# Kakekakechan/AKBRaytracing

Hardware: AMD Instinct MI355X
Metric: ray-surface intersections/sec + PSF wall-time, 1e7-ray 4-mirror AKB, 1/2/4/8 GPU (higher is better)
Workload: dtype f64

## Files before the change

akbraytracing_amd/_lib.py:

```python
import atexit
import ctypes
import os

import torch

from . import build as _build

_LIB = None

c_i32 = ctypes.c_int32
c_i64 = ctypes.c_int64
c_int = ctypes.c_int
c_dbl = ctypes.c_double
c_vp = ctypes.c_void_p
MAX_MIRRORS = 7
ABI_VERSION = 19

FLAG_MISS = 0x1
FLAG_ZERO_NORMAL = 0x2
FLAG_ZERO_REFLECT = 0x4
FLAG_ZERO_DIR = 0x8
FLAG_CHAIN_DIR = 1 << 28
FLAG_FIG_OUTSIDE = 0x8

EXPORTS = [
    "akb_last_error", "akb_abi_version", "akb_sources_hash", "akb_device_count",
    "akb_stream_create_reserved", "akb_stream_destroy", "akb_reserved_cu_mask",
    "akb_isect_f64", "akb_normal_f64", "akb_reflect_f64", "akb_normalize_f64", "akb_plane_isect_f64",
    "akb_seglen_f64", "akb_rotate_f64", "akb_fill_nan_f64",
    "akb_isect_dd_f64", "akb_reflect_dd_f64", "akb_trace_chain_dd_f64", "akb_figure_opl_f64", "akb_figure_normal_f64",
    "akb_trace_chain_f64", "akb_chain_desc_size", "akb_tilt_opd_f64", "akb_tilt_params_f64",
    "akb_tilt_opd_dev_f64", "akb_chain_tilt_f64", "akb_chain_tilt_opd_f64", "akb_trace_chain_samples_f64", "akb_opd_f64", "akb_resample_f64", "akb_plane_sweep_rows_f64",
    "akb_plane_sweep_sink_f64",
    "akb_calc_ds_f64",
    "akb_pairwise_work_bytes", "akb_pairwise_sum_f64", "akb_pupil_sample_f64",
    "akb_leaf_sink_bytes", "akb_leaf_sink_layout", "akb_leaf_finish_work_bytes", "akb_leaf_finish_f64",
    "akb_leaf_parts_f64", "akb_parts_chain_f64",
    "akb_huygens_splits", "akb_huygens_work_bytes", "akb_huygens_f64", "akb_scale_field_f64",
    "akb_psf_work_bytes", "akb_psf_f64", "akb_psf_release_plans", "akb_release_all", "akb_selftest_arith_f64",
    "akb_first_valid_rows_f64", "akb_rotate_work_bytes", "akb_rotate_with_nan_f64", "akb_pupil_post_f64", "akb_pupil_post_work_bytes",
    "akb_moments_work_bytes", "akb_map_moments_f64", "akb_plane_subtract_f64", "akb_legendre_rows_f64",
    "akb_gd_cells_f64", "akb_gd_pockets", "akb_gd_check_pockets", "akb_gd_grad_sweeps_f64",
    "akb_gd_eval_f64", "akb_gd_cone_work_bytes", "akb_gd_patch_timing", "akb_gd_patch_times", "akb_gd_band_times", "akb_gd_patch_phases", "akb_gd_patch_order", "akb_gd_cone_eval_f64", "akb_gd_axes_f64",
    "akb_gd_cells_claims_f64", "akb_gd_claim_pockets_f64", "akb_gd_cone_solve_f64",
    "akb_gd_claims_f64", "akb_gd_cone_part_f64", "akb_gd_part_finish_f64", "akb_gd_ring_f64", "akb_gd_cells_window_f64",
    "akb_trace_chain_batch_f64", "akb_focus_eval_work_bytes", "akb_focus_eval_f64", "akb_sep_search_f64",
    "akb_finish_params_work_bytes", "akb_finish_tilt_params_f64",
    "akb_valid_mask_u8", "akb_external_contours", "akb_approx_poly_dp", "akb_affine_from_points",
    "akb_affine_invert", "akb_warp_affine_f64",
]


class LeafSink(ctypes.Structure):
    _fields_ = [
        ("leaf_sum", c_vp), ("leaf_cnt", c_vp), ("tail", c_vp),
        ("nq", c_i32), ("nan_mask", c_i32), ("n", c_i64),
    ]


class FigureMapDesc(ctypes.Structure):
    _fields_ = [
        ("table", c_vp),
        ("origin", c_dbl * 3), ("e_u", c_dbl * 3), ("e_w", c_dbl * 3),
        ("u0", c_dbl), ("du", c_dbl), ("w0", c_dbl), ("dw", c_dbl),
        ("nu", c_i32), ("nw", c_i32),
    ]

# ... 124 lines not shown
        "akb_gd_grad_sweeps_f64": ([c_vp, c_vp, c_int, c_int, c_vp, c_int, c_vp, c_vp, c_vp, c_vp, c_vp, c_vp, c_int,
                                    c_vp, c_vp, c_dbl, c_dbl, c_int, c_vp, c_vp, c_vp, c_vp, c_vp], c_int),
        "akb_gd_eval_f64": ([c_vp, c_vp, c_int, c_int, c_vp, c_int, c_vp, c_vp, c_vp, c_vp, c_int, c_vp, c_int,
                             c_vp, c_vp, c_int, c_vp, c_vp, c_vp], c_int),
        "akb_gd_cone_work_bytes": ([c_int, c_int, c_int, c_int, c_int], c_i64),
        "akb_gd_patch_timing": ([c_int], c_int),
        "akb_gd_patch_order": ([c_int, c_vp], c_int),
        "akb_gd_patch_times": ([c_vp, c_vp, c_int], c_int),
        "akb_gd_band_times": ([c_vp, c_int], c_int),
        "akb_gd_patch_phases": ([c_vp], c_int),
        "akb_gd_axes_f64": ([c_vp, c_vp, c_i64, c_int, c_int, c_vp, c_vp, c_vp, c_vp], c_int),
        "akb_gd_claims_f64": ([c_vp, c_vp, c_int, c_int, c_vp, c_int, c_vp, c_vp, c_vp, c_int, c_int, c_int, c_vp,
                               c_int, c_vp, c_int, c_vp, c_vp, c_vp], c_int),
        "akb_gd_cone_part_f64": ([c_vp, c_vp, c_int, c_int, c_vp, c_int, c_vp, c_vp, c_vp, c_vp, c_vp, c_i64, c_i64,
                                  c_int, c_vp, c_int, c_vp, c_int, c_vp, c_int, c_int, c_vp, c_vp, c_vp, c_vp, c_vp,
                                  c_vp, c_vp], c_int),
        "akb_gd_part_finish_f64": ([c_vp, c_vp, c_i64, c_int, c_vp], c_int),
        "akb_gd_ring_f64": ([c_vp, c_vp, c_int, c_int, c_vp, c_vp, c_vp, c_vp], c_int),
        "akb_gd_cells_window_f64": ([c_vp, c_vp, c_int, c_int, c_int, c_int, c_vp, c_dbl, c_vp, c_vp], c_int),
        "akb_gd_cone_eval_f64": ([c_vp, c_vp, c_int, c_int, c_vp, c_int, c_vp, c_vp, c_vp, c_vp, c_vp, c_vp, c_int,
                                  c_vp, c_int, c_vp, c_int, c_int, c_vp, c_vp, c_vp, c_vp, c_vp, c_vp], c_int),
        "akb_gd_cone_solve_f64": ([c_vp, c_vp, c_int, c_int, c_vp, c_int, c_vp, c_vp, c_vp, c_vp, c_vp, c_vp, c_int,
                                   c_vp, c_int, c_vp, c_int, c_int, c_vp, c_vp, c_vp, c_vp, c_vp, c_vp], c_int),
        "akb_gd_cells_claims_f64": ([c_vp, c_vp, c_int, c_int, c_vp, c_dbl, c_vp, c_vp, c_int, c_vp, c_int, c_vp,
                                     c_vp], c_int),
        "akb_gd_claim_pockets_f64": ([c_vp, c_vp, c_int, c_int, c_vp, c_int, c_vp, c_vp, c_int, c_vp, c_int, c_vp,
                                      c_vp], c_int),
    }
    for name, (args, res) in sig.items():
        try:
            f = getattr(L, name)
        except AttributeError:
            raise AKBError(f"the library lacks {name}: it was built from other sources, rebuild "
                           "(python -m akbraytracing_amd.build)") from None
        f.argtypes = args
        f.restype = res


def lib():
    global _LIB
    if _LIB is None:
        path = os.environ.get("AKB_LIB") or _build.SO
        if not os.path.exists(path):
            raise AKBError(
                f"{path} is missing: build the HIP extension first (python -m akbraytracing_amd.build "
                "or __graft_entry__.build()); there is no CPU fallback")
# ... 33 lines not shown
```

akbraytracing_amd/csrc/akb_griddata.hip:

```cpp
#include <hip/hip_runtime.h>
#include <math.h>
#include <stdint.h>
#include <stdio.h>

#include <algorithm>
#include <mutex>
#include <type_traits>

#include "akb_common.h"
#include "akb_pairwise.h"

namespace akb {
namespace {

struct Grid {
    const double* x;
    const double* y;
    int nv, nh;
    const uint8_t* diag;
    int npock;
    const int32_t* ptri;
    const int32_t* pnbr;
    const int32_t* edge_tri;
    const int32_t* xptr;
// ... 438 lines not shown
    }
    for (int off = 32; off > 0; off >>= 1) acc |= __shfl_down(acc, off);
    if (lane == 0) {
        const unsigned cur = __hip_atomic_load(flags, __ATOMIC_RELAXED, __HIP_MEMORY_SCOPE_AGENT);
        if ((cur | acc) != cur) atomicOr(flags, acc);
    }
}

__global__ void k_gd_ring(Grid g, double* rx, double* ry, unsigned* flags) {
    AKB_CHAIN_PRIORITY();
    const int64_t a = g.nh - 1, b = g.nv - 1, L = 2 * a + 2 * b;
    for (int64_t r = blockIdx.x * (int64_t)blockDim.x + threadIdx.x; r < L; r += (int64_t)gridDim.x * blockDim.x) {
        int64_t v;
        if (r < a) v = r;
        else if (r < a + b) v = (r - a) * g.nh + (g.nh - 1);
        else if (r < 2 * a + b) v = (int64_t)(g.nv - 1) * g.nh + (g.nh - 1 - (r - a - b));
        else v = (int64_t)(g.nv - 1 - (r - 2 * a - b)) * g.nh;
        rx[r] = g.x[v];
        ry[r] = g.y[v];
        if (!isfinite(rx[r]) || !isfinite(ry[r])) atomicOr(flags, 32u);
    }
}

__global__ void k_gd_check_pockets(Grid g, double tol, unsigned* flags) {
    AKB_CHAIN_PRIORITY();
    const int64_t nc2 = 2 * ncells(g);
    for (int64_t j = blockIdx.x * (int64_t)blockDim.x + threadIdx.x; j < g.npock; j += (int64_t)gridDim.x * blockDim.x) {
        const Tri T = tri_verts(g, nc2 + j);
        for (int k = 0; k < 3; ++k) {
            const int64_t n = tri_nbr(g, nc2 + j, k);
            if (n < 0) continue;
            const Tri N = tri_verts(g, n);
            int64_t o = -1;
            for (int q = 0; q < 3; ++q)
                if (N.v[q] != T.v[(k + 1) % 3] && N.v[q] != T.v[(k + 2) % 3]) o = N.v[q];
            if (o < 0) {
                atomicOr(flags, 4u);
                continue;
            }
            const double x0 = g.x[T.v[0]], y0 = g.y[T.v[0]];
            const double bx = g.x[T.v[1]] - x0, by = g.y[T.v[1]] - y0, cx = g.x[T.v[2]] - x0, cy = g.y[T.v[2]] - y0;
            const double ox = g.x[o] - x0, oy = g.y[o] - y0;
            const double s = fmax(fmax(fabs(bx), fabs(by)), fmax(fmax(fabs(cx), fabs(cy)), fmax(fabs(ox), fabs(oy))));
            if (incircle(0.0, 0.0, bx, by, cx, cy, ox, oy) > tol * s * s * s * s) atomicOr(flags, 2u);
        }
    }
}


__device__ __forceinline__ int64_t ring_pos(const Grid& g, int iv, int ih) {
    const int64_t a = g.nh - 1, b = g.nv - 1;
    if (iv == 0) return ih;
    if (ih == g.nh - 1) return a + iv;
    if (iv == g.nv - 1) return a + b + (g.nh - 1 - ih);
    if (ih == 0) return 2 * a + b + (g.nv - 1 - iv);
    return -1;
}

__device__ __forceinline__ int64_t ring_vertex(const Grid& g, int64_t r) {
    const int64_t ra = g.nh - 1, rb = g.nv - 1;
    if (r < ra) return r;
    if (r < ra + rb) return (r - ra) * g.nh + (g.nh - 1);
    if (r < 2 * ra + rb) return (int64_t)(g.nv - 1) * g.nh + (g.nh - 1 - (r - ra - rb));
    return (int64_t)(g.nv - 1 - (r - 2 * ra - rb)) * g.nh;
}

struct EdgeG {
    double mxx, mxy, myy, wx, wy;
};
// ... 688 lines not shown
        int32_t* sr = slots + r * kChordSlots;
        for (int k = 0; k < kChordSlots; ++k)
            sr[k] = cnt > kChordSlots ? kSlotBig
                    : k >= cnt        ? -1
                    : cnt > 8         ? -g.xidx[k0 + k] - 3
                                      : g.xidx[k0 + k];
    }
}

constexpr int kBandThreads = 256, kBandRingWaves = kBandThreads / 64, kBandRingPer = 8 * kBandRingWaves;
constexpr int kBandTileThreads = kBandThreads, kBandVR = kBandTR * kBandTC / kBandTileThreads;
__device__ __forceinline__ void band_clock(unsigned long long* clk, int k, unsigned long long t0) {
    __syncthreads();
    if (threadIdx.x == 0) {
        const unsigned long long d = wall_clock64() - t0;
        atomicAdd(&clk[2 * k], d);
        atomicAdd(&clk[2 * k + 1], 1ull);
        atomicMax(&clk[4 + k], d);
    }
}
inline unsigned band_ring_wgs(int64_t L) { return (unsigned)((L + kBandRingPer - 1) / kBandRingPer); }
inline unsigned band_grid(const BandTiles& bt, int64_t L) { return band_ring_wgs(L) + (unsigned)bt.total; }

__global__ void __launch_bounds__(kBandThreads) __attribute__((amdgpu_waves_per_eu(4))) k_gd_cone_band(Grid g, BandTiles bt, ConeBand a) {
    AKB_CHAIN_PRIORITY();
    if (!*a.needed) return;
    const unsigned long long t0 = a.clk ? wall_clock64() : 0;
    constexpr int HR = kBandTR + 2, HC = kBandTC + 2, HN = HR * HC, CC = kBandTC + 1;
    __shared__ double sx[HN], sy[HN], sf[HN], sgx[HN], sgy[HN];
    __shared__ double spx[kBandTR * kBandTC], spy[kBandTR * kBandTC];
    __shared__ uint8_t sdg[(kBandTR + 1) * CC];
    const int64_t L = 2 * (int64_t)(g.nh - 1) + 2 * (int64_t)(g.nv - 1);
    const int nr = (int)((L + kBandRingPer - 1) / kBandRingPer);
    const int w = threadIdx.x >> 6, lane = threadIdx.x & 63;
    if ((int)blockIdx.x < nr) {
        const int sub = lane & 7;
        const int64_t q0 = (int64_t)blockIdx.x * kBandRingPer + 8 * w;
        const int64_t r = q0 + (lane >> 3);
        int32_t js[4] = {-1, -1, -1, -1};
        bool big;
        if (a.slots) {
            if (r < L) {
#pragma unroll
                for (int k = 0; k < 4; ++k) js[k] = a.slots[r * kChordSlots + sub + 8 * k];
            }
            big = js[0] == kSlotBig;
        } else {
            big = r < L && g.xptr[r + 1] - g.xptr[r] > 8;
        }
        if (r < L && !big) cone_ring_vertex<8>(g, a, r, sub, js);
        unsigned long long m = __ballot(big && sub == 0);
        while (m) {
            const int q = __builtin_ctzll(m);
            m &= m - 1;
            cone_ring_vertex<64>(g, a, q0 + (q >> 3), lane);
        }
        if (a.clk) band_clock(a.clk + 4, 0, t0);
        return;
    }
    int r0 = 0, c0 = 0, r1 = 0, c1 = 0;
    band_tile(bt, g.nv, g.nh, (int)blockIdx.x - nr, r0, c0, r1, c1);
    {
        constexpr int NQ = (HN + kBandThreads - 1) / kBandThreads, NC = ((kBandTR + 1) * CC + kBandThreads - 1) / kBandThreads;
        constexpr int NP = kBandTR * kBandTC / kBandThreads;
        double lx[NQ], ly[NQ], lf[NQ], lgx[NQ], lgy[NQ], lpx[NP], lpy[NP];
        uint8_t ld[NC];
#pragma unroll
        for (int u = 0; u < NQ; ++u) {
            const int k = threadIdx.x + u * kBandThreads;
            const int iv = r0 - 1 + k / HC, ih = c0 - 1 + (k - (k / HC) * HC);
            lx[u] = ly[u] = lf[u] = lgx[u] = lgy[u] = 0.0;
            if (k < HN && iv >= 0 && iv < g.nv && ih >= 0 && ih < g.nh) {
                const int64_t q = (int64_t)iv * g.nh + ih;
                lx[u] = g.x[q];
                ly[u] = g.y[q];
                lf[u] = a.f[q];
                lgx[u] = a.gin ? a.gin[2 * q] : 0.0;
                lgy[u] = a.gin ? a.gin[2 * q + 1] : 0.0;
            }
        }
#pragma unroll
        for (int u = 0; u < NC; ++u) {
            const int k = threadIdx.x + u * kBandThreads;
            const int cv = r0 - 1 + k / CC, ch = c0 - 1 + (k - (k / CC) * CC);
// ... 49 lines not shown
        const int lc = tr * CC + tc;
        const int dc[4] = {lc, lc + 1, lc + CC, lc + CC + 1};
        uint8_t dg[4];
#pragma unroll
        for (int k = 0; k < 4; ++k) dg[k] = inb[4 + k] ? sdg[dc[k]] : 0;
        double xs[8], ys[8], fs[8], gxs[8], gys[8];
#pragma unroll
        for (int k = 0; k < 8; ++k) {
            const int j = inb[k] ? jn[k] : li;
            xs[k] = sx[j];
            ys[k] = sy[j];
            fs[k] = sf[j];
            gxs[k] = sgx[j];
            gys[k] = sgy[j];
        }
        const bool on[8] = {L_, R, D, U, inb[4] && dg[0] == 0, inb[5] && dg[1] == 1, inb[6] && dg[2] == 1,
                            inb[7] && dg[3] == 0};
        GradAcc<1> A;
        band_edges(A, sx[li], sy[li], sf[li], xs, ys, fs, gxs, gys, on);
        const int pk = tr * kBandTC + tc;
        band_solve(a, (int64_t)iv * g.nh + ih, A, spx[pk], spy[pk]);
    }
    if (a.clk) band_clock(a.clk + 4, 1, t0);
}

struct ConePatch {
    const double* f;
    const int64_t* cells;
    const int* count;
    int K;
    ConeStep st[kConeMaxK + 1];
    double* gout;
    unsigned long long* chg;
    unsigned long long* est;
    unsigned long long* clk;
};

__constant__ uint16_t c_patch_order[kConeMaxK + 1][1024];

inline int b128_lane_group(int lane) {
    const int x = lane & 31;
    const bool first = x < 4 || (x >= 12 && x < 16) || (x >= 20 && x < 28);
    return (lane >> 5) * 2 + (first ? 0 : 1);
}

inline void patch_order_table(int K, int S, uint16_t* out) {
// ... 446 lines not shown
    __shared__ PwTree tree[2];
    __threadfence_block();
    __syncthreads();
    const int w = threadIdx.x >> 6;
    if (w < 2) {
        const long long cnt = (long long)mx * my;
        const double* a = lds ? (w == 0 ? sgx : sgy) : (w == 0 ? gx : gy);
        const int m = w == 0 ? mx : my;
        double sum;
        sum = pw_sum_wave_get(tree[w], MeshgridAxis{a, mx, w == 0}, cnt);
        const double mean = sum / (double)cnt;
        if ((threadIdx.x & 63) == 0) ext[4 + w] = m > 1 ? fabs((a[1] - mean) - (a[0] - mean)) : 0.0;
    }
}

__device__ __forceinline__ bool cone_interior(const Grid& g, int o, int K, int64_t& c, int64_t& p00) {
    if (o >= 2 * ncells(g)) return false;
    c = o >> 1;
    const int iv = (int)(c / (g.nh - 1)), ih = (int)(c - (int64_t)iv * (g.nh - 1));
    p00 = (int64_t)iv * g.nh + ih;
    return iv - K - 1 >= 1 && iv + K + 2 <= g.nv - 2 && ih - K - 1 >= 1 && ih + K + 2 <= g.nh - 2;
}

__global__ void __launch_bounds__(kBlock) k_gd_cone_assign(Grid g, const int* __restrict__ owner, int64_t m, int K,
                                                            int64_t own0, int64_t own1, int band_on, int64_t* cells,
                                                            int* count, int* band, uint8_t* assigned) {
    AKB_CHAIN_PRIORITY();
    for (int64_t t = blockIdx.x * (int64_t)blockDim.x + threadIdx.x; t < m; t += (int64_t)gridDim.x * blockDim.x) {
        const int o = owner[t];
        uint8_t mine = 0;
        if (o != INT32_MAX) {
            int64_t c = -1, p00 = -1;
            const bool interior = cone_interior(g, o, K, c, p00);
            if (interior) {
                if (p00 >= own0 && p00 < own1) {
                    cells[atomicAdd(count, 1)] = c;
                    mine = 1;
                }
            } else if (band_on) {
                atomicOr(band, 1);
                mine = 1;
            }
        }
        assigned[t] = mine;
    }
}

__global__ void __launch_bounds__(kBlock) k_gd_claim(Grid g, Targets t, int* owner) {
    AKB_CHAIN_PRIORITY();
    const int64_t ntri = 2 * ncells(g);
    for (int64_t id = blockIdx.x * (int64_t)blockDim.x + threadIdx.x; id < ntri; id += (int64_t)gridDim.x * blockDim.x) {
        const Tri T = tri_verts(g, id);
        int c0, c1, r0, r1;
        tri_box(g, t, T, c0, c1, r0, r1);
        for (int r = r0; r < r1; ++r)
            for (int c = c0; c < c1; ++c) claim_one(g, t, T, (int)id, r, c, owner);
    }
}

__device__ __forceinline__ void claim_cell(const Grid& g, const Targets& t, int64_t c, bool uniform, double inv_dx,
                                           double inv_dy, int* owner) {
    const int iv = (int)(c / (g.nh - 1)), ih = (int)(c - (int64_t)iv * (g.nh - 1));
    const int64_t p00 = (int64_t)iv * g.nh + ih;
    const double xa = g.x[p00], xb = g.x[p00 + 1], xc = g.x[p00 + g.nh], xd = g.x[p00 + g.nh + 1];
    const double ya = g.y[p00], yb = g.y[p00 + 1], yc = g.y[p00 + g.nh], yd = g.y[p00 + g.nh + 1];
    const double xlo = fmin(fmin(xa, xb), fmin(xc, xd)), xhi = fmax(fmax(xa, xb), fmax(xc, xd));
    const double ylo = fmin(fmin(ya, yb), fmin(yc, yd)), yhi = fmax(fmax(ya, yb), fmax(yc, yd));
    const double padx = (xhi - xlo) * 1e-9, pady = (yhi - ylo) * 1e-9;
// ... 159 lines not shown
    Targets tl = t;
    if (t.mx <= kClaimAxisLds && t.my <= kClaimAxisLds) {
        for (int i = threadIdx.x; i < t.mx; i += blockDim.x) sax[i] = t.gx[i];
        for (int i = threadIdx.x; i < t.my; i += blockDim.x) sax[kClaimAxisLds + i] = t.gy[i];
        __syncthreads();
        tl.gx = sax;
        tl.gy = sax + kClaimAxisLds;
    }
    const int lane = threadIdx.x & 63, wv = threadIdx.x >> 6, nw = blockDim.x >> 6;
    int64_t nblk;
    int bh, r_lo, r_hi;
    claim_block_dims(g, nblk, bh, r_lo, r_hi);
    for (int64_t blk = (int64_t)blockIdx.x * nw + wv; blk < nblk; blk += (int64_t)gridDim.x * nw) {
        if (!hit[blk]) continue;
        const int bv = (int)(blk / bh), bc = (int)(blk - (int64_t)bv * bh);
        const int iv0 = r_lo + bv * 8, ih0 = bc * 8;
        const int nr = min(8, r_hi - iv0), nc = min(8, g.nh - 1 - ih0);
        const int rr = lane >> 3, cc = lane & 7;
        if (rr < nr && cc < nc) claim_cell(g, tl, (int64_t)(iv0 + rr) * (g.nh - 1) + (ih0 + cc), uniform, inv_dx, inv_dy,
                                           owner);
    }
}

__global__ void __launch_bounds__(kBlock) k_gd_claim_pockets(Grid g, Targets t, int* owner) {
    AKB_CHAIN_PRIORITY();
    const int64_t nc2 = 2 * ncells(g);
    const int lane = threadIdx.x & 63, nw = blockDim.x >> 6;
    __shared__ double sax[2 * kClaimAxisLds];
    if (t.mx <= kClaimAxisLds && t.my <= kClaimAxisLds) {
        for (int i = threadIdx.x; i < t.mx; i += blockDim.x) sax[i] = t.gx[i];
        for (int i = threadIdx.x; i < t.my; i += blockDim.x) sax[kClaimAxisLds + i] = t.gy[i];
        __syncthreads();
        t.gx = sax;
        t.gy = sax + kClaimAxisLds;
    }
    for (int64_t j = (int64_t)blockIdx.x * nw + (threadIdx.x >> 6); j < g.npock; j += (int64_t)gridDim.x * nw) {
        const Tri T = tri_verts(g, nc2 + j);
        int c0, c1, r0, r1;
        tri_box(g, t, T, c0, c1, r0, r1);
        const int w = c1 - c0;
        const int64_t m = (int64_t)w * (r1 - r0);
        for (int64_t k = lane; k < m; k += 64) {
            const int r = r0 + (int)(k / w), c = c0 + (int)(k - (int64_t)(k / w) * w);
            claim_one(g, t, T, (int)(nc2 + j), r, c, owner);
        }
    }
}

struct CTIn {
    double px[3], py[3], f[3], gx[3], gy[3];
    double cx[3], cy[3];
    bool nb[3];
};

__device__ __forceinline__ void bary_v(const double (&x)[3], const double (&y)[3], double px, double py,
                                       double (&b)[3]) {
    const double x2 = x[2], y2 = y[2];
    const double a00 = x[0] - x2, a01 = x[1] - x2;
    const double a10 = y[0] - y2, a11 = y[1] - y2;
    const double det = a00 * a11 - a01 * a10;
    const double t00 = a11 / det, t01 = -a01 / det, t10 = -a10 / det, t11 = a00 / det;
    const double dx = px - x2, dy = py - y2;
    b[0] = t00 * dx + t01 * dy;
    b[1] = t10 * dx + t11 * dy;
    b[2] = 1.0 - b[0] - b[1];
}

__device__ double ct_eval(const CTIn& in, const double (&b)[3]) {
    const double p0x = in.px[0], p0y = in.py[0];
// ... 414 lines not shown
    AKB_REQUIRE(ring_x && ring_y && gx && gy && L > 0 && mx > 0 && my > 0, "bad arguments");
    k_gd_axes<<<1, kAxesThreads, 0, (hipStream_t)stream>>>(ring_x, ring_y, L, mx, my, gx, gy, d_extent);
    return launch_status("k_gd_axes");
}


static int64_t claim_scratch_bytes(int nv, int nh) {
    return ((int64_t)((nv - 1 + 7) / 8) * ((nh - 1 + 7) / 8) + 63) / 64 * 64;
}
static int64_t claim_scratch_offset(int nv, int nh, int mx, int my, int nvals) {
    const int64_t n = (int64_t)nv * nh, L = 2 * (int64_t)(nh - 1) + 2 * (int64_t)(nv - 1);
    const int nv2 = nvals >= 2 ? 2 : 1;
    const int64_t m = (int64_t)mx * my;
    return (3 * (int64_t)nv2 * n * 2 * 8 + L * 16 * 8 + m * 8 + m + 64 + 63) / 64 * 64;
}

int64_t akb_gd_cone_work_bytes(int nv, int nh, int mx, int my, int nvals) {
    if (nv < 2 || nh < 2 || mx < 1 || my < 1 || nvals < 1) return -1;
    return claim_scratch_offset(nv, nh, mx, my, nvals) + claim_scratch_bytes(nv, nh);
}

namespace {

int cone_claims(const Grid& g, const Targets& t, int with_pockets, int* owner, hipStream_t s, uint8_t* scratch = nullptr) {
    const int64_t m = (int64_t)t.mx * t.my;
    k_fill_i32<<<grid_for(m, 4), kBlock, 0, s>>>(owner, m, INT32_MAX);
    int st = launch_status("k_fill_i32");
    if (st) return st;
    const int64_t wc = (int64_t)((g.row1 < 0 ? g.nv - 1 : g.row1) - g.row0) * (g.nh - 1);
    if (wc > 0) {
        if (scratch) {
            const int64_t nblk = (int64_t)(((g.row1 < 0 ? g.nv - 1 : g.row1) - g.row0 + 7) / 8) * ((g.nh - 1 + 7) / 8);
            k_gd_claim_scan<<<grid_for(nblk, 1, kStreamGridCap), kBlock, 0, s>>>(g, t, scratch);
            if ((st = launch_status("k_gd_claim_scan"))) return st;
            k_gd_claim_hit<<<grid_for(nblk * 16, 1, kStreamGridCap), kBlock, 0, s>>>(g, t, scratch, owner);
        } else {
            k_gd_claim_blocks<<<grid_for(wc / 16 + 1, 1, kStreamGridCap), kBlock, 0, s>>>(g, t, owner);
        }
        if ((st = launch_status("k_gd_claim"))) return st;
    }
    if (with_pockets && g.npock > 0) {
        const int64_t pw = ((int64_t)g.npock + kBlock / 64 - 1) / (kBlock / 64);
        k_gd_claim_pockets<<<(unsigned)(pw < 16384 ? pw : 16384), kBlock, 0, s>>>(g, t, owner);
        if ((st = launch_status("k_gd_claim_pockets"))) return st;
    }
    return 0;
}

int cone_part(const Grid& g, const Targets& t, int64_t own0, int64_t own1, int band_on, const double* f, int nvals,
              int K, const double* omegas, void* work, const int* owner, double* out, double* cnt,
              unsigned long long* d_change, hipStream_t s) {
    const int64_t n = (int64_t)g.nv * g.nh, m = (int64_t)t.mx * t.my;
    const int64_t L = 2 * (int64_t)(g.nh - 1) + 2 * (int64_t)(g.nv - 1);
    double* gb[3];
    for (int k = 0; k < 3; ++k) gb[k] = (double*)work + (int64_t)k * n * 2;
    const int nv2 = nvals >= 2 ? 2 : 1;
    int64_t* cells = (int64_t*)((double*)work + 3 * (int64_t)nv2 * n * 2 + L * 16);
    uint8_t* assigned = (uint8_t*)(cells + m);
    int* count = (int*)(((uintptr_t)(assigned + m) + 7) & ~(uintptr_t)7);
    int* band = count + 1;
    if (hipMemsetAsync(count, 0, 2 * sizeof(int), s) != hipSuccess) return launch_status("hipMemsetAsync");
    k_gd_cone_assign<<<grid_for(m, 1), kBlock, 0, s>>>(g, owner, m, K, own0, own1, band_on, cells, count, band,
                                                      assigned);
    int st = launch_status("k_gd_cone_assign");
    if (st) return st;
    ConeStep steps[kConeMaxK + 1];
    steps[0] = ConeStep{0, 1.0};
    for (int j = 1; j <= K; ++j)
        steps[j] = j == 1 ? ConeStep{0, 1.0} : j == 2 ? ConeStep{1, omegas[1]} : ConeStep{2, omegas[j - 1]};
    const int S = patch_split(K);
    const unsigned pp = gd_cu_count();
    AKB_REQUIRE(S >= 0 && m <= 1024 * (int64_t)pp, "cone patches: K or the target count out of range");
    if (patch_order_upload(s)) {
        set_error("cone patches: the vertex order table did not reach constant memory");
        return AKB_E_HIP;
    }
    for (int v = 0; v < nvals; ++v) {
        const double* fv = f + v * n;
        if (band_on) {
            PatchTimer& bt0 = patch_timer();
            const int bslot = (int)(bt0.band_launches % kPatchEvents);
            if (bt0.on) (void)hipEventRecord(bt0.bev[bslot][0], s);
            int32_t* slots = (int32_t*)((double*)work + 3 * (int64_t)nv2 * n * 2);
            if (v == 0) {
                k_gd_chord_slots<<<grid_for(L), kBlock, 0, s>>>(g, slots, L);
                if ((st = launch_status("k_gd_chord_slots"))) return st;
            }
            for (int j = 1; j <= K; ++j) {
                const double* gin = j == 1 ? nullptr : gb[(j - 1) % 3];
                const double* gprev = j >= 3 ? gb[(j + 1) % 3] : nullptr;
                const BandTiles bt = band_tiles(g.nv, g.nh, 2 * K + 3 - j);
                const ConeBand a{fv, gin, gprev, gb[j % 3], steps[j], band, patch_timer().band_clk ? patch_timer().clk : nullptr,
                                 slots};
                k_gd_cone_band<<<band_grid(bt, L), kBandThreads, 0, s>>>(g, bt, a);
                if ((st = launch_status("k_gd_cone_band"))) return st;
            }
            if (d_change) {
                const BandTiles bt = band_tiles(g.nv, g.nh, K + 2);
                const ConeBand a{fv, gb[K % 3], nullptr, gb[(K + 1) % 3], ConeStep{0, 1.0}, band,
                                 patch_timer().band_clk ? patch_timer().clk : nullptr, slots};
                k_gd_cone_band<<<band_grid(bt, L), kBandThreads, 0, s>>>(g, bt, a);
                if ((st = launch_status("k_gd_cone_band"))) return st;
            }
            if (bt0.on) {
                (void)hipEventRecord(bt0.bev[bslot][1], s);
                ++bt0.band_launches;
            }
        }
        const BandEst be{band_on && d_change ? gb[(K + 1) % 3] : nullptr, K, d_change, d_change ? d_change + 1 : nullptr};
        ConePatch a{fv, cells, count, K, {}, gb[K % 3], d_change, d_change ? d_change + 1 : nullptr,
                    patch_timer().on ? patch_timer().clk : nullptr};
        for (int j = 0; j <= K; ++j) a.st[j] = steps[j];
        PatchTimer& pt = patch_timer();
        const int slot = (int)(pt.launches % kPatchEvents);
        if (pt.on) {
            (void)hipEventRecord(pt.ev[slot][0], s);
            pt.cnt[slot] = count;
// ... 64 lines not shown
    const int64_t pw = ((int64_t)npock + kBlock / 64 - 1) / (kBlock / 64);
    k_gd_claim_pockets<<<(unsigned)(pw < 16384 ? pw : 16384), kBlock, 0, (hipStream_t)stream>>>(g, Targets{gx, gy, mx, my},
                                                                                               owner);
    return launch_status("k_gd_claim_pockets");
}

int akb_gd_cone_solve_f64(const double* x, const double* y, int nv, int nh, const uint8_t* diag, int npock,
                          const int32_t* ptri, const int32_t* pnbr, const int32_t* edge_tri, const int32_t* xptr,
                          const int32_t* xidx, const double* gx, int mx, const double* gy, int my, const double* f,
                          int nvals, int K, const double* omegas, void* work, const int* owner, double* out,
                          unsigned long long* d_change, void* stream) {
    clear_error();
    AKB_REQUIRE(x && y && diag && gx && gy && f && omegas && work && owner && out && mx > 0 && my > 0 && nvals >= 1,
                "bad arguments");
    AKB_REQUIRE(K >= 1 && K <= kConeMaxK, "K sweeps in 1 .. 14");
    AKB_REQUIRE(nv >= 2 && nh >= 2, "grid of at least 2 x 2 points");
    AKB_REQUIRE(xptr && xidx && (npock == 0 || (ptri && pnbr && edge_tri)), "the band needs the pockets");
    for (int j = 2; j <= K; ++j) AKB_REQUIRE(omegas[j - 1] > 0 && omegas[j - 1] < 2, "Chebyshev weight outside (0, 2)");
    Grid g{x, y, nv, nh, diag, npock, ptri, pnbr, edge_tri, xptr, xidx};
    return cone_part(g, Targets{gx, gy, mx, my}, 0, (int64_t)nv * nh, 1, f, nvals, K, omegas, work, owner, out, nullptr,
                     d_change, (hipStream_t)stream);
}

int akb_gd_claims_f64(const double* x, const double* y, int nv, int nh, const uint8_t* diag, int npock,
                      const int32_t* ptri, const int32_t* pnbr, const int32_t* edge_tri, int row0, int row1,
                      int with_pockets, const double* gx, int mx, const double* gy, int my, int* owner, void* work,
                      void* stream) {
    clear_error();
    AKB_REQUIRE(x && y && diag && gx && gy && owner && mx > 0 && my > 0, "bad arguments");
    AKB_REQUIRE(nv >= 2 && nh >= 2 && row0 >= 0 && row1 <= nv - 1 && (row1 < 0 || row0 <= row1), "bad window");
    AKB_REQUIRE(!with_pockets || npock == 0 || (ptri && pnbr && edge_tri), "pockets needed");
    Grid g{x, y, nv, nh, diag, npock, ptri, pnbr, edge_tri, nullptr, nullptr};
    g.row0 = row0;
    g.row1 = row1;
    return cone_claims(g, Targets{gx, gy, mx, my}, with_pockets, owner, (hipStream_t)stream,
                       work ? (uint8_t*)work + claim_scratch_offset(nv, nh, mx, my, 1) : nullptr);
}

int akb_gd_cone_part_f64(const double* x, const double* y, int nv, int nh, const uint8_t* diag, int npock,
                         const int32_t* ptri, const int32_t* pnbr, const int32_t* edge_tri, const int32_t* xptr,
                         const int32_t* xidx, int64_t own0, int64_t own1, int band_on, const double* gx, int mx,
                         const double* gy, int my, const double* f, int nvals, int K, const double* omegas, void* work,
                         const int* owner, double* out, double* cnt, unsigned long long* d_change, void* stream) {
    clear_error();
    AKB_REQUIRE(x && y && diag && gx && gy && f && omegas && work && owner && out && cnt && mx > 0 && my > 0,
                "bad arguments");
// ... 124 lines not shown
```

akbraytracing_amd/faithful.py:

```python
import concurrent.futures
import time

import numpy as np
import torch

from . import _lib
from . import device as D
from .griddata import CONE_GUARD, CONE_SWEEPS, ConeNotConverged, CubicGrid, build_pockets, chebyshev_weights
from .griddata import pocket_offsets, raise_for_cell_flags, raise_for_pocket_status
from .psf import image_axes, psf_stack
from .pupilmap import POST_PARAMS, pupil_post, pupil_post_check

EUV = 13.5e-9


def pack_pockets(buf, o, Lr):
    npk = int(buf[o["npk"]])
    nx = int(buf[o["xptr"] + Lr])
    nbr = buf[o["nbr"]:o["nbr"] + 3 * npk].copy()
    rest = np.concatenate([buf[o["edge"]:o["edge"] + Lr], buf[o["xptr"]:o["xptr"] + Lr + 1],
                           buf[o["xidx"]:o["xidx"] + nx]])
    p = dict(tri=0, nbr=3 * npk, edge=6 * npk, xptr=6 * npk + Lr, xidx=6 * npk + 2 * Lr + 1)
    assert o["tri"] == 0
    buf[p["nbr"]:p["nbr"] + 3 * npk] = nbr
# ... 202 lines not shown
            t.npock = D.wait_result(t.job)
        except BaseException:
            t.y = t.z = t.f = None
            t.finished = True
            raise
        s = t.slot
        st = stream_of(stream)
        sh = D.stream_handle(st)
        o, Lr = s["po"], self.L
        with torch.cuda.stream(st):
            if self._done is not None:
                st.wait_event(self._done)
            if events is not None:
                events[0].record(st)
            s["pk"][:o["len"]].copy_(s["pk_host"][:o["len"]], non_blocking=True)
            t.h2d = torch.cuda.Event()
            t.h2d.record(st)
            pk = s["pk"]
            k = max(t.npock, 1)
            ptri, pnbr = pk[o["tri"]:o["tri"] + 3 * k], pk[o["nbr"]:o["nbr"] + 3 * k]
            edge, xptr, xidx = pk[o["edge"]:o["edge"] + Lr], pk[o["xptr"]:o["xptr"] + Lr + 1], pk[o["xidx"]:o["len"] + 1]
            tri = (D.ptr(t.y), D.ptr(t.z), self.nv, self.nh, D.ptr(s["diag"]), t.npock, D.ptr(ptri), D.ptr(pnbr),
                   D.ptr(edge))
            self.words[:3].zero_()
            _lib.check(L.akb_gd_check_pockets(*tri, self.tol, D.ptr(self.status), sh))
            m = self.size
            axes = s["axes"]
            gx, gy = axes[:m], axes[m:2 * m]
            _lib.check(L.akb_gd_claim_pockets_f64(D.ptr(t.y), D.ptr(t.z), self.nv, self.nh, D.ptr(s["diag"]), t.npock,
                                                  D.ptr(ptri), D.ptr(gx), m, D.ptr(gy), m, D.ptr(s["owner"]), sh))
            _lib.check(L.akb_gd_cone_solve_f64(*tri, D.ptr(xptr), D.ptr(xidx), D.ptr(gx), m, D.ptr(gy), m,
                                               D.ptr(t.f), 1, self.sweeps, self._omegas, D.ptr(self.work),
                                               D.ptr(s["owner"]), D.ptr(self.map), D.ptr(self.change), sh))
            t.result = self._post_psf(st, axes, psf_events, post_events)
            if events is not None:
                events[1].record(st)
            t.erow = self.errors.record((self.words,), st)
            t.done = self._end(st)
        t.y = t.z = t.f = None
        t.finished = True
        self.finished += 1
        return t.result

    def run(self, y, z, f, stream=None):
        t = self.begin(y, z, f, stream)
        r = self.finish(t, stream)
        try:
            t.check()
        except ConeNotConverged:
            r = self._converged(y, z, f, t.slot["axes"], stream)
        return r

    def _converged(self, y, z, f, ax, stream=None):
        st = stream_of(stream)
        m = self.size
        with torch.cuda.stream(st):
# ... 16 lines not shown
```

include/akb_raytrace.h:

```cpp
#ifndef AKB_RAYTRACE_H
#define AKB_RAYTRACE_H

#include <stdint.h>

#ifdef __cplusplus
extern "C" {
#endif

#define AKB_ABI_VERSION 19

#define AKB_OK 0
#define AKB_E_INVALID (-1)
#define AKB_E_HIP (-2)
#define AKB_E_FFT (-3)
#define AKB_E_NOMEM (-4)
#define AKB_E_ARG AKB_E_INVALID

#define AKB_FLAG_MISS 0x1
#define AKB_FLAG_ZERO_NORMAL 0x2
#define AKB_FLAG_ZERO_REFLECT 0x4
#define AKB_FLAG_ZERO_DIR 0x8
#define AKB_FLAG_CHAIN_DIR (1 << 28)
#define AKB_FLAG_FIG_OUTSIDE 0x8

// ... 240 lines not shown
int akb_gd_patch_timing(int enable);
int akb_gd_patch_times(float* ms, int* cells, int max);
int akb_gd_band_times(float* ms, int max);
int akb_gd_patch_phases(unsigned long long* out);
int akb_gd_patch_order(int K, uint16_t* out);
int akb_gd_axes_f64(const double* ring_x, const double* ring_y, int64_t L, int mx, int my, double* gx, double* gy,
                    double* d_extent, void* stream);
int akb_gd_cone_eval_f64(const double* x, const double* y, int nv, int nh, const uint8_t* diag, int npock,
                         const int32_t* ptri, const int32_t* pnbr, const int32_t* edge_tri, const int32_t* xptr,
                         const int32_t* xidx, const double* gx, int mx, const double* gy, int my, const double* f,
                         int nvals, int K, const double* omegas, void* work, int* owner, double* out,
                         unsigned long long* d_change, void* stream);
int akb_gd_cells_claims_f64(const double* x, const double* y, int nv, int nh, uint8_t* diag, double tol,
                            unsigned* d_flags, const double* gx, int mx, const double* gy, int my, int* owner,
                            void* stream);
int akb_gd_claim_pockets_f64(const double* x, const double* y, int nv, int nh, const uint8_t* diag, int npock,
                             const int32_t* ptri, const double* gx, int mx, const double* gy, int my, int* owner,
                             void* stream);
int akb_gd_cone_solve_f64(const double* x, const double* y, int nv, int nh, const uint8_t* diag, int npock,
                          const int32_t* ptri, const int32_t* pnbr, const int32_t* edge_tri, const int32_t* xptr,
                          const int32_t* xidx, const double* gx, int mx, const double* gy, int my, const double* f,
                          int nvals, int K, const double* omegas, void* work, const int* owner, double* out,
                          unsigned long long* d_change, void* stream);

int akb_gd_cells_window_f64(const double* x, const double* y, int nv, int nh, int row0, int row1, uint8_t* diag,
                            double tol, unsigned* d_flags, void* stream);
int akb_gd_ring_f64(const double* x, const double* y, int nv, int nh, double* ring_x, double* ring_y, unsigned* d_flags,
                    void* stream);
int akb_gd_claims_f64(const double* x, const double* y, int nv, int nh, const uint8_t* diag, int npock,
                      const int32_t* ptri, const int32_t* pnbr, const int32_t* edge_tri, int row0, int row1,
                      int with_pockets, const double* gx, int mx, const double* gy, int my, int* owner, void* work,
                      void* stream);
int akb_gd_cone_part_f64(const double* x, const double* y, int nv, int nh, const uint8_t* diag, int npock,
                         const int32_t* ptri, const int32_t* pnbr, const int32_t* edge_tri, const int32_t* xptr,
                         const int32_t* xidx, int64_t own0, int64_t own1, int band_on, const double* gx, int mx,
                         const double* gy, int my, const double* f, int nvals, int K, const double* omegas, void* work,
                         const int* owner, double* out, double* cnt, unsigned long long* d_change, void* stream);
int akb_gd_part_finish_f64(double* out, const double* cnt, int64_t m, int nvals, void* stream);

#define AKB_SELFTEST_COLS 13
int akb_selftest_arith_f64(const double* a, const double* b, int64_t n, double* out, void* stream);

void akb_psf_release_plans(void);

void akb_release_all(void);

// ... 6 lines not shown
```

Before: 58.79 billion.

## Fold pocket check, pocket claims and cone assign into leading band-sweep launches

Adds a cone_finish entry point that merges the pocket-consistency check, pocket claiming, chord-slot fill, status/count zeroing and cone assignment into extra leading workgroups of the first two k_gd_cone_band launches. Python now calls this single entry instead of three separate library calls. The aim is to remove several small kernel launches and memsets, and the gaps between them, on the griddata path. In exchange the band kernels carry a templated lead path, and the code relies on the work in each launch being independent. The claims in launch 1 must finish before the assign in launch 2 reads the owner array, which kernel order on the stream provides.

```diff
diff --git a/akbraytracing_amd/_lib.py b/akbraytracing_amd/_lib.py
--- a/akbraytracing_amd/_lib.py
+++ b/akbraytracing_amd/_lib.py
@@ -42,7 +42,7 @@
     "akb_moments_work_bytes", "akb_map_moments_f64", "akb_plane_subtract_f64", "akb_legendre_rows_f64",
     "akb_gd_cells_f64", "akb_gd_pockets", "akb_gd_check_pockets", "akb_gd_grad_sweeps_f64",
     "akb_gd_eval_f64", "akb_gd_cone_work_bytes", "akb_gd_patch_timing", "akb_gd_patch_times", "akb_gd_band_times", "akb_gd_patch_phases", "akb_gd_patch_order", "akb_gd_cone_eval_f64", "akb_gd_axes_f64",
-    "akb_gd_cells_claims_f64", "akb_gd_claim_pockets_f64", "akb_gd_cone_solve_f64",
+    "akb_gd_cells_claims_f64", "akb_gd_claim_pockets_f64", "akb_gd_cone_solve_f64", "akb_gd_cone_finish_f64",
     "akb_gd_claims_f64", "akb_gd_cone_part_f64", "akb_gd_part_finish_f64", "akb_gd_ring_f64", "akb_gd_cells_window_f64",
     "akb_trace_chain_batch_f64", "akb_focus_eval_work_bytes", "akb_focus_eval_f64", "akb_sep_search_f64",
     "akb_finish_params_work_bytes", "akb_finish_tilt_params_f64",
@@ -213,6 +213,9 @@
                                   c_vp, c_int, c_vp, c_int, c_int, c_vp, c_vp, c_vp, c_vp, c_vp, c_vp], c_int),
         "akb_gd_cone_solve_f64": ([c_vp, c_vp, c_int, c_int, c_vp, c_int, c_vp, c_vp, c_vp, c_vp, c_vp, c_vp, c_int,
                                    c_vp, c_int, c_vp, c_int, c_int, c_vp, c_vp, c_vp, c_vp, c_vp, c_vp], c_int),
+        "akb_gd_cone_finish_f64": ([c_vp, c_vp, c_int, c_int, c_vp, c_int, c_vp, c_vp, c_vp, c_vp, c_vp, c_dbl, c_vp,
+                                    c_vp, c_int, c_vp, c_int, c_vp, c_int, c_int, c_vp, c_vp, c_vp, c_vp, c_vp, c_vp],
+                                   c_int),
         "akb_gd_cells_claims_f64": ([c_vp, c_vp, c_int, c_int, c_vp, c_dbl, c_vp, c_vp, c_int, c_vp, c_int, c_vp,
                                      c_vp], c_int),
         "akb_gd_claim_pockets_f64": ([c_vp, c_vp, c_int, c_int, c_vp, c_int, c_vp, c_vp, c_int, c_vp, c_int, c_vp,
diff --git a/akbraytracing_amd/csrc/akb_griddata.hip b/akbraytracing_amd/csrc/akb_griddata.hip
--- a/akbraytracing_amd/csrc/akb_griddata.hip
+++ b/akbraytracing_amd/csrc/akb_griddata.hip
@@ -484,10 +484,9 @@
     }
 }
 
-__global__ void k_gd_check_pockets(Grid g, double tol, unsigned* flags) {
-    AKB_CHAIN_PRIORITY();
+__device__ __forceinline__ void check_pockets_part(const Grid& g, double tol, unsigned* flags, unsigned b, unsigned nb) {
     const int64_t nc2 = 2 * ncells(g);
-    for (int64_t j = blockIdx.x * (int64_t)blockDim.x + threadIdx.x; j < g.npock; j += (int64_t)gridDim.x * blockDim.x) {
+    for (int64_t j = b * (int64_t)blockDim.x + threadIdx.x; j < g.npock; j += (int64_t)nb * blockDim.x) {
         const Tri T = tri_verts(g, nc2 + j);
         for (int k = 0; k < 3; ++k) {
             const int64_t n = tri_nbr(g, nc2 + j, k);
@@ -507,6 +506,10 @@
             if (incircle(0.0, 0.0, bx, by, cx, cy, ox, oy) > tol * s * s * s * s) atomicOr(flags, 2u);
         }
     }
+}
+__global__ void k_gd_check_pockets(Grid g, double tol, unsigned* flags) {
+    AKB_CHAIN_PRIORITY();
+    check_pockets_part(g, tol, flags, blockIdx.x, gridDim.x);
 }
 
 
@@ -1241,9 +1244,31 @@
 inline unsigned band_ring_wgs(int64_t L) { return (unsigned)((L + kBandRingPer - 1) / kBandRingPer); }
 inline unsigned band_grid(const BandTiles& bt, int64_t L) { return band_ring_wgs(L) + (unsigned)bt.total; }
 
-__global__ void __launch_bounds__(kBandThreads) __attribute__((amdgpu_waves_per_eu(4))) k_gd_cone_band(Grid g, BandTiles bt, ConeBand a) {
+struct BandLead {
+    unsigned nrid;
+    unsigned long long* status;
+    unsigned long long* change;
+    int* count;
+    Targets t;
+    int* owner;
+    int32_t* slots;
+    double tol;
+    unsigned ncheck;
+    int64_t m, own0, own1;
+    int K, band_on;
+    int64_t* cells;
+    uint8_t* assigned;
+};
+__device__ __forceinline__ void check_pockets_part(const Grid& g, double tol, unsigned* flags, unsigned b, unsigned nb);
+__device__ __forceinline__ void claim_pockets_part(const Grid& g, const Targets& t, int* owner, unsigned b, unsigned nb);
+__device__ __forceinline__ void cone_assign_part(const Grid& g, const int* __restrict__ owner, int64_t m, int K,
+                                                 int64_t own0, int64_t own1, int band_on, int64_t* cells, int* count,
+                                                 int* band, uint8_t* assigned, unsigned b, unsigned nb);
+
+template <int kLead>
+__device__ __forceinline__ void cone_band_body(const Grid g, const BandTiles bt, const ConeBand a, const BandLead* ld) {
     AKB_CHAIN_PRIORITY();
-    if (!*a.needed) return;
+    if (kLead == 0 && !*a.needed) return;
     const unsigned long long t0 = a.clk ? wall_clock64() : 0;
     constexpr int HR = kBandTR + 2, HC = kBandTC + 2, HN = HR * HC, CC = kBandTC + 1;
     __shared__ double sx[HN], sy[HN], sf[HN], sgx[HN], sgy[HN];
@@ -1252,12 +1277,49 @@
     const int64_t L = 2 * (int64_t)(g.nh - 1) + 2 * (int64_t)(g.nv - 1);
     const int nr = (int)((L + kBandRingPer - 1) / kBandRingPer);
     const int w = threadIdx.x >> 6, lane = threadIdx.x & 63;
-    if ((int)blockIdx.x < nr) {
+    const unsigned nrid = kLead ? ld->nrid : 0u;
+    if (kLead && blockIdx.x < nrid) {
+        if (kLead == 1) {
+            if (blockIdx.x == 0) {
+                if (threadIdx.x == 0) *ld->status = 0ull;
+                if (threadIdx.x == 1 || threadIdx.x == 2) ld->change[threadIdx.x - 1] = 0ull;
+                if (threadIdx.x == 3 || threadIdx.x == 4) ld->count[threadIdx.x - 3] = 0;
+                return;
+            }
+            Targets t = ld->t;
+            if (t.mx <= kClaimAxisLds && t.my <= kClaimAxisLds) {
+                static_assert(HN >= kClaimAxisLds, "the claims' axes lie over sx and sy");
+                for (int i = threadIdx.x; i < t.mx; i += kBandThreads) sx[i] = t.gx[i];
+                for (int i = threadIdx.x; i < t.my; i += kBandThreads) sy[i] = t.gy[i];
+                __syncthreads();
+                t.gx = sx;
+                t.gy = sy;
+            }
+            claim_pockets_part(g, t, ld->owner, blockIdx.x - 1, nrid - 1);
+        } else if (blockIdx.x < ld->ncheck) {
+            check_pockets_part(g, ld->tol, (unsigned*)ld->status, blockIdx.x, ld->ncheck);
+        } else {
+            cone_assign_part(g, ld->owner, ld->m, ld->K, ld->own0, ld->own1, ld->band_on, ld->cells, ld->count,
+                             ld->count + 1, ld->assigned, blockIdx.x - ld->ncheck, nrid - ld->ncheck);
+        }
+        return;
+    }
+    const unsigned wg = blockIdx.x - nrid;
+    if ((int)wg < nr) {
         const int sub = lane & 7;
-        const int64_t q0 = (int64_t)blockIdx.x * kBandRingPer + 8 * w;
+        const int64_t q0 = (int64_t)wg * kBandRingPer + 8 * w;
         const int64_t r = q0 + (lane >> 3);
         int32_t js[4] = {-1, -1, -1, -1};
         bool big;
+        if (kLead == 1 && r < L) {
+            const int32_t k0 = g.xptr[r], cnt = g.xptr[r + 1] - k0;
+#pragma unroll
+            for (int k = sub; k < kChordSlots; k += 8)
+                ld->slots[r * kChordSlots + k] = cnt > kChordSlots ? kSlotBig
+                                                 : k >= cnt        ? -1
+                                                 : cnt > 8         ? -g.xidx[k0 + k] - 3
+                                                                   : g.xidx[k0 + k];
+        }
         if (a.slots) {
             if (r < L) {
 #pragma unroll
@@ -1278,7 +1340,7 @@
         return;
     }
     int r0 = 0, c0 = 0, r1 = 0, c1 = 0;
-    band_tile(bt, g.nv, g.nh, (int)blockIdx.x - nr, r0, c0, r1, c1);
+    band_tile(bt, g.nv, g.nh, (int)wg - nr, r0, c0, r1, c1);
     {
         constexpr int NQ = (HN + kBandThreads - 1) / kBandThreads, NC = ((kBandTR + 1) * CC + kBandThreads - 1) / kBandThreads;
         constexpr int NP = kBandTR * kBandTC / kBandThreads;
@@ -1374,6 +1436,14 @@
         band_solve(a, (int64_t)iv * g.nh + ih, A, spx[pk], spy[pk]);
     }
     if (a.clk) band_clock(a.clk + 4, 1, t0);
+}
+
+__global__ void __launch_bounds__(kBandThreads) __attribute__((amdgpu_waves_per_eu(4))) k_gd_cone_band(Grid g, BandTiles bt, ConeBand a) {
+    cone_band_body<0>(g, bt, a, nullptr);
+}
+template <int kLead>
+__global__ void __launch_bounds__(kBandThreads) __attribute__((amdgpu_waves_per_eu(4))) k_gd_cone_band_lead(Grid g, BandTiles bt, ConeBand a, BandLead ld) {
+    cone_band_body<kLead>(g, bt, a, &ld);
 }
 
 struct ConePatch {
@@ -1866,11 +1936,10 @@
     return iv - K - 1 >= 1 && iv + K + 2 <= g.nv - 2 && ih - K - 1 >= 1 && ih + K + 2 <= g.nh - 2;
 }
 
-__global__ void __launch_bounds__(kBlock) k_gd_cone_assign(Grid g, const int* __restrict__ owner, int64_t m, int K,
-                                                            int64_t own0, int64_t own1, int band_on, int64_t* cells,
-                                                            int* count, int* band, uint8_t* assigned) {
-    AKB_CHAIN_PRIORITY();
-    for (int64_t t = blockIdx.x * (int64_t)blockDim.x + threadIdx.x; t < m; t += (int64_t)gridDim.x * blockDim.x) {
+__device__ __forceinline__ void cone_assign_part(const Grid& g, const int* __restrict__ owner, int64_t m, int K,
+                                                 int64_t own0, int64_t own1, int band_on, int64_t* cells, int* count,
+                                                 int* band, uint8_t* assigned, unsigned b, unsigned nb) {
+    for (int64_t t = b * (int64_t)blockDim.x + threadIdx.x; t < m; t += (int64_t)nb * blockDim.x) {
         const int o = owner[t];
         uint8_t mine = 0;
         if (o != INT32_MAX) {
@@ -1888,6 +1957,12 @@
         }
         assigned[t] = mine;
     }
+}
+__global__ void __launch_bounds__(kBlock) k_gd_cone_assign(Grid g, const int* __restrict__ owner, int64_t m, int K,
+                                                            int64_t own0, int64_t own1, int band_on, int64_t* cells,
+                                                            int* count, int* band, uint8_t* assigned) {
+    AKB_CHAIN_PRIORITY();
+    cone_assign_part(g, owner, m, K, own0, own1, band_on, cells, count, band, assigned, blockIdx.x, gridDim.x);
 }
 
 __global__ void __launch_bounds__(kBlock) k_gd_claim(Grid g, Targets t, int* owner) {
@@ -2093,19 +2168,10 @@
     }
 }
 
-__global__ void __launch_bounds__(kBlock) k_gd_claim_pockets(Grid g, Targets t, int* owner) {
-    AKB_CHAIN_PRIORITY();
+__device__ __forceinline__ void claim_pockets_part(const Grid& g, const Targets& t, int* owner, unsigned b, unsigned nb) {
     const int64_t nc2 = 2 * ncells(g);
     const int lane = threadIdx.x & 63, nw = blockDim.x >> 6;
-    __shared__ double sax[2 * kClaimAxisLds];
-    if (t.mx <= kClaimAxisLds && t.my <= kClaimAxisLds) {
-        for (int i = threadIdx.x; i < t.mx; i += blockDim.x) sax[i] = t.gx[i];
-        for (int i = threadIdx.x; i < t.my; i += blockDim.x) sax[kClaimAxisLds + i] = t.gy[i];
-        __syncthreads();
-        t.gx = sax;
-        t.gy = sax + kClaimAxisLds;
-    }
-    for (int64_t j = (int64_t)blockIdx.x * nw + (threadIdx.x >> 6); j < g.npock; j += (int64_t)gridDim.x * nw) {
+    for (int64_t j = (int64_t)b * nw + (threadIdx.x >> 6); j < g.npock; j += (int64_t)nb * nw) {
         const Tri T = tri_verts(g, nc2 + j);
         int c0, c1, r0, r1;
         tri_box(g, t, T, c0, c1, r0, r1);
@@ -2116,6 +2182,18 @@
             claim_one(g, t, T, (int)(nc2 + j), r, c, owner);
         }
     }
+}
+__global__ void __launch_bounds__(kBlock) k_gd_claim_pockets(Grid g, Targets t, int* owner) {
+    AKB_CHAIN_PRIORITY();
+    __shared__ double sax[2 * kClaimAxisLds];
+    if (t.mx <= kClaimAxisLds && t.my <= kClaimAxisLds) {
+        for (int i = threadIdx.x; i < t.mx; i += blockDim.x) sax[i] = t.gx[i];
+        for (int i = threadIdx.x; i < t.my; i += blockDim.x) sax[kClaimAxisLds + i] = t.gy[i];
+        __syncthreads();
+        t.gx = sax;
+        t.gy = sax + kClaimAxisLds;
+    }
+    claim_pockets_part(g, t, owner, blockIdx.x, gridDim.x);
 }
 
 struct CTIn {
@@ -2576,6 +2654,11 @@
 
 namespace {
 
+inline unsigned claim_pockets_grid(int npock) {
+    const int64_t pw = ((int64_t)npock + kBlock / 64 - 1) / (kBlock / 64);
+    return (unsigned)(pw < 16384 ? pw : 16384);
+}
+
 int cone_claims(const Grid& g, const Targets& t, int with_pockets, int* owner, hipStream_t s, uint8_t* scratch = nullptr) {
     const int64_t m = (int64_t)t.mx * t.my;
     k_fill_i32<<<grid_for(m, 4), kBlock, 0, s>>>(owner, m, INT32_MAX);
@@ -2601,9 +2684,14 @@
     return 0;
 }
 
+struct ConeFinish {
+    unsigned long long* status;
+    double tol;
+    int* owner;
+};
 int cone_part(const Grid& g, const Targets& t, int64_t own0, int64_t own1, int band_on, const double* f, int nvals,
               int K, const double* omegas, void* work, const int* owner, double* out, double* cnt,
-              unsigned long long* d_change, hipStream_t s) {
+              unsigned long long* d_change, hipStream_t s, const ConeFinish* fin = nullptr) {
     const int64_t n = (int64_t)g.nv * g.nh, m = (int64_t)t.mx * t.my;
     const int64_t L = 2 * (int64_t)(g.nh - 1) + 2 * (int64_t)(g.nv - 1);
     double* gb[3];
@@ -2613,11 +2701,25 @@
     uint8_t* assigned = (uint8_t*)(cells + m);
     int* count = (int*)(((uintptr_t)(assigned + m) + 7) & ~(uintptr_t)7);
     int* band = count + 1;
-    if (hipMemsetAsync(count, 0, 2 * sizeof(int), s) != hipSuccess) return launch_status("hipMemsetAsync");
-    k_gd_cone_assign<<<grid_for(m, 1), kBlock, 0, s>>>(g, owner, m, K, own0, own1, band_on, cells, count, band,
-                                                      assigned);
-    int st = launch_status("k_gd_cone_assign");
-    if (st) return st;
+    const bool lead = fin && K >= 2 && band_on && d_change;
+    int st = 0;
+    if (fin && !lead) {
+        if (hipMemsetAsync(fin->status, 0, sizeof(unsigned long long), s) != hipSuccess ||
+            (d_change && hipMemsetAsync(d_change, 0, 2 * sizeof(unsigned long long), s) != hipSuccess))
+            return launch_status("hipMemsetAsync");
+        if (g.npock > 0) {
+            k_gd_check_pockets<<<grid_for(g.npock), kBlock, 0, s>>>(g, fin->tol, (unsigned*)fin->status);
+            if ((st = launch_status("k_gd_check_pockets"))) return st;
+            k_gd_claim_pockets<<<claim_pockets_grid(g.npock), kBlock, 0, s>>>(g, t, fin->owner);
+            if ((st = launch_status("k_gd_claim_pockets"))) return st;
+        }
+    }
+    if (!lead) {
+        if (hipMemsetAsync(count, 0, 2 * sizeof(int), s) != hipSuccess) return launch_status("hipMemsetAsync");
+        k_gd_cone_assign<<<grid_for(m, 1), kBlock, 0, s>>>(g, owner, m, K, own0, own1, band_on, cells, count, band,
+                                                          assigned);
+        if ((st = launch_status("k_gd_cone_assign"))) return st;
+    }
     ConeStep steps[kConeMaxK + 1];
     steps[0] = ConeStep{0, 1.0};
     for (int j = 1; j <= K; ++j)
@@ -2636,7 +2738,7 @@
             const int bslot = (int)(bt0.band_launches % kPatchEvents);
             if (bt0.on) (void)hipEventRecord(bt0.bev[bslot][0], s);
             int32_t* slots = (int32_t*)((double*)work + 3 * (int64_t)nv2 * n * 2);
-            if (v == 0) {
+            if (v == 0 && !lead) {
                 k_gd_chord_slots<<<grid_for(L), kBlock, 0, s>>>(g, slots, L);
                 if ((st = launch_status("k_gd_chord_slots"))) return st;
             }
@@ -2645,8 +2747,17 @@
                 const double* gprev = j >= 3 ? gb[(j + 1) % 3] : nullptr;
                 const BandTiles bt = band_tiles(g.nv, g.nh, 2 * K + 3 - j);
                 const ConeBand a{fv, gin, gprev, gb[j % 3], steps[j], band, patch_timer().band_clk ? patch_timer().clk : nullptr,
-                                 slots};
-                k_gd_cone_band<<<band_grid(bt, L), kBandThreads, 0, s>>>(g, bt, a);
+                                 lead && v == 0 && j == 1 ? nullptr : slots};
+                if (lead && v == 0 && j <= 2) {
+                    const unsigned nclaim = g.npock > 0 ? claim_pockets_grid(g.npock) : 0u;
+                    const unsigned ncheck = g.npock > 0 ? grid_for(g.npock) : 0u;
+                    const BandLead ld{j == 1 ? 1 + nclaim : ncheck + grid_for(m, 1), fin->status, d_change, count, t,
+                                      fin->owner, slots, fin->tol, ncheck, m, own0, own1, K, band_on, cells, assigned};
+                    if (j == 1) k_gd_cone_band_lead<1><<<ld.nrid + band_grid(bt, L), kBandThreads, 0, s>>>(g, bt, a, ld);
+                    else k_gd_cone_band_lead<2><<<ld.nrid + band_grid(bt, L), kBandThreads, 0, s>>>(g, bt, a, ld);
+                } else {
+                    k_gd_cone_band<<<band_grid(bt, L), kBandThreads, 0, s>>>(g, bt, a);
+                }
                 if ((st = launch_status("k_gd_cone_band"))) return st;
             }
             if (d_change) {
@@ -2757,6 +2868,25 @@
                      d_change, (hipStream_t)stream);
 }
 
+int akb_gd_cone_finish_f64(const double* x, const double* y, int nv, int nh, const uint8_t* diag, int npock,
+                           const int32_t* ptri, const int32_t* pnbr, const int32_t* edge_tri, const int32_t* xptr,
+                           const int32_t* xidx, double tol, unsigned long long* d_status, const double* gx, int mx,
+                           const double* gy, int my, const double* f, int nvals, int K, const double* omegas, void* work,
+                           int* owner, double* out, unsigned long long* d_change, void* stream) {
+    clear_error();
+    AKB_REQUIRE(x && y && diag && gx && gy && f && omegas && work && owner && out && mx > 0 && my > 0 && nvals >= 1,
+                "bad arguments");
+    AKB_REQUIRE(d_status && d_change, "the status word and the change words");
+    AKB_REQUIRE(K >= 1 && K <= kConeMaxK, "K sweeps in 1 .. 14");
+    AKB_REQUIRE(nv >= 2 && nh >= 2, "grid of at least 2 x 2 points");
+    AKB_REQUIRE(xptr && xidx && (npock == 0 || (ptri && pnbr && edge_tri)), "the band needs the pockets");
+    for (int j = 2; j <= K; ++j) AKB_REQUIRE(omegas[j - 1] > 0 && omegas[j - 1] < 2, "Chebyshev weight outside (0, 2)");
+    Grid g{x, y, nv, nh, diag, npock, ptri, pnbr, edge_tri, xptr, xidx};
+    const ConeFinish fin{d_status, tol, owner};
+    return cone_part(g, Targets{gx, gy, mx, my}, 0, (int64_t)nv * nh, 1, f, nvals, K, omegas, work, owner, out, nullptr,
+                     d_change, (hipStream_t)stream, &fin);
+}
+
 int akb_gd_claims_f64(const double* x, const double* y, int nv, int nh, const uint8_t* diag, int npock,
                       const int32_t* ptri, const int32_t* pnbr, const int32_t* edge_tri, int row0, int row1,
                       int with_pockets, const double* gx, int mx, const double* gy, int my, int* owner, void* work,
diff --git a/akbraytracing_amd/faithful.py b/akbraytracing_amd/faithful.py
--- a/akbraytracing_amd/faithful.py
+++ b/akbraytracing_amd/faithful.py
@@ -248,16 +248,13 @@
             edge, xptr, xidx = pk[o["edge"]:o["edge"] + Lr], pk[o["xptr"]:o["xptr"] + Lr + 1], pk[o["xidx"]:o["len"] + 1]
             tri = (D.ptr(t.y), D.ptr(t.z), self.nv, self.nh, D.ptr(s["diag"]), t.npock, D.ptr(ptri), D.ptr(pnbr),
                    D.ptr(edge))
-            self.words[:3].zero_()
-            _lib.check(L.akb_gd_check_pockets(*tri, self.tol, D.ptr(self.status), sh))
             m = self.size
             axes = s["axes"]
             gx, gy = axes[:m], axes[m:2 * m]
-            _lib.check(L.akb_gd_claim_pockets_f64(D.ptr(t.y), D.ptr(t.z), self.nv, self.nh, D.ptr(s["diag"]), t.npock,
-                                                  D.ptr(ptri), D.ptr(gx), m, D.ptr(gy), m, D.ptr(s["owner"]), sh))
-            _lib.check(L.akb_gd_cone_solve_f64(*tri, D.ptr(xptr), D.ptr(xidx), D.ptr(gx), m, D.ptr(gy), m,
-                                               D.ptr(t.f), 1, self.sweeps, self._omegas, D.ptr(self.work),
-                                               D.ptr(s["owner"]), D.ptr(self.map), D.ptr(self.change), sh))
+            _lib.check(L.akb_gd_cone_finish_f64(*tri, D.ptr(xptr), D.ptr(xidx), self.tol, D.ptr(self.status),
+                                                D.ptr(gx), m, D.ptr(gy), m, D.ptr(t.f), 1, self.sweeps, self._omegas,
+                                                D.ptr(self.work), D.ptr(s["owner"]), D.ptr(self.map),
+                                                D.ptr(self.change), sh))
             t.result = self._post_psf(st, axes, psf_events, post_events)
             if events is not None:
                 events[1].record(st)
diff --git a/include/akb_raytrace.h b/include/akb_raytrace.h
--- a/include/akb_raytrace.h
+++ b/include/akb_raytrace.h
@@ -286,6 +286,11 @@
                           const int32_t* xidx, const double* gx, int mx, const double* gy, int my, const double* f,
                           int nvals, int K, const double* omegas, void* work, const int* owner, double* out,
                           unsigned long long* d_change, void* stream);
+int akb_gd_cone_finish_f64(const double* x, const double* y, int nv, int nh, const uint8_t* diag, int npock,
+                           const int32_t* ptri, const int32_t* pnbr, const int32_t* edge_tri, const int32_t* xptr,
+                           const int32_t* xidx, double tol, unsigned long long* d_status, const double* gx, int mx,
+                           const double* gy, int my, const double* f, int nvals, int K, const double* omegas, void* work,
+                           int* owner, double* out, unsigned long long* d_change, void* stream);
 
 int akb_gd_cells_window_f64(const double* x, const double* y, int nv, int nh, int row0, int row1, uint8_t* diag,
                             double tol, unsigned* d_flags, void* stream);
```

Result: slower. 57.81 billion (-1.7%).
